# superlinear-ai/raglite

Measured on AMD Instinct MI355X. Metric: queries/sec, MaxSim 32x1M d=1024 exact top-100, higher is better.
Workload: dtype f32 in / f32 scores: candidate chunks found with the fp16 hi halves of corpus and queries (1 x v_mfma_f32_16x16x32_f16 per multiply, f32 accumulate, rigorous error bound), their scores by v_mfma_f32_16x16x4_f32 (exact f32 products); full-precision fallback: 3 x v_mfma_f32_16x16x32_f16 on hi+lo pairs

## Files before the change

### raglite_amd/csrc/maxsim_pp.hip

```cpp
#include <cstdio>
#include <cstdlib>
#include <utility>

#include "common.h"
#include "pp_schedule.h"

namespace rl {

typedef float f32x4 __attribute__((ext_vector_type(4)));
typedef _Float16 h16x8 __attribute__((ext_vector_type(8)));

namespace {
constexpr int PP_RT = 128;
constexpr int PP_NBLK = PP_RT / 16;
constexpr int PP_QPP = 16;
constexpr int PP_DC = 8;
constexpr int PP_LC = 6;
constexpr int PP_CSLOT = PP_NBLK * 1024;
constexpr int PP_STAGE = 1536;
constexpr int PP_LDS = PP_DC * PP_CSLOT + 16 * PP_STAGE * 4;

__device__ __forceinline__ int64_t pp_uniform_i64(int64_t v) {
    const uint32_t lo = __builtin_amdgcn_readfirstlane((uint32_t)(uint64_t)v);
    const uint32_t hi = __builtin_amdgcn_readfirstlane((uint32_t)((uint64_t)v >> 32));
    return (int64_t)(((uint64_t)hi << 32) | lo);
}

enum { PP_HINT_NONE = 0, PP_HINT_NT = 1, PP_HINT_SC1 = 2 };
template <bool NT>
__device__ __forceinline__ void pp_dma(uint32_t lds, const char* src, uint32_t lane16, int hint) {
    const uint32_t l = __builtin_amdgcn_readfirstlane(lds);
    const char* const p = reinterpret_cast<const char*>(pp_uniform_i64(reinterpret_cast<int64_t>(src)));
#ifdef RAGLITE_EXPERIMENTS
    if (!NT && hint == PP_HINT_SC1) {
        asm volatile("s_mov_b32 m0, %0\n\ts_nop 0\n\tglobal_load_lds_dwordx4 %1, %2 sc1" ::"s"(l), "v"(lane16), "s"(p) : "memory", "m0");
        return;
    }
    if (NT || hint == PP_HINT_NT)
#else
    if constexpr (NT)
#endif
        asm volatile("s_mov_b32 m0, %0\n\ts_nop 0\n\tglobal_load_lds_dwordx4 %1, %2 nt" ::"s"(l), "v"(lane16), "s"(p) : "memory", "m0");
    else
        asm volatile("s_mov_b32 m0, %0\n\ts_nop 0\n\tglobal_load_lds_dwordx4 %1, %2" ::"s"(l), "v"(lane16), "s"(p) : "memory", "m0");
}

template <int OFF>
__device__ __forceinline__ void pp_read(f32x4& dst, uint32_t addr) {
    asm volatile("ds_read_b128 %0, %1 offset:%2" : "=v"(dst) : "v"(addr), "n"(OFF) : "memory");
}
__device__ __forceinline__ void pp_pin(f32x4& a, f32x4& b, f32x4& c, f32x4& d) { asm volatile("" : "+v"(a), "+v"(b), "+v"(c), "+v"(d)); }
typedef float f32x16s __attribute__((ext_vector_type(16)));
__device__ __forceinline__ f32x16s pp_sload16(const float* p) {
    f32x16s v;
    const float* const u = reinterpret_cast<const float*>(pp_uniform_i64(reinterpret_cast<int64_t>(p)));
    asm volatile("s_load_dwordx16 %0, %1, 0x0\n\ts_waitcnt lgkmcnt(0)" : "=s"(v) : "s"(u) : "memory");
    return v;
}
__device__ __forceinline__ h16x8 pp_h(const f32x4& v) {
    h16x8 r;
    __builtin_memcpy(&r, &v, 16);
    return r;
}
}

struct PpRows {
    const float* tau;
    const float* q_unscale;
    const float* q_sumsq;
    const float* row_norm;
    const float* blk_minmax;
    int32_t B, QT, metric;
    float* cand_scores; int32_t* cand_ids; uint32_t* cand_cnt; uint32_t* overflow; int32_t cap;
    uint2* log; int32_t log_cap;
    int32_t tile_begin, tile_count;
    float* S; int64_t ld_s; int32_t stride;
    int32_t xcd_passes, dma_hint;
};

template <int DBG, int MODE, bool ROWNORM>
__global__ __launch_bounds__(512, 2) void maxsim_pp_kernel(const char* __restrict__ planes, int64_t n_rows, int32_t nslab,
                                                           const char* __restrict__ qfrag, const float* __restrict__ qmeta, int32_t n_q,
                                                           const int32_t* __restrict__ row_to_chunk, const int64_t* __restrict__ chunk_offsets,
                                                           const uint32_t* __restrict__ ends_bits, float* __restrict__ out, int64_t out_stride,
                                                           float inv_e_scale, const uint32_t* __restrict__ run_if, PpRows rs) {
    constexpr bool ROWS = MODE == 2, SCORES = MODE == 1, GROUPS = ROWS || SCORES;
    __shared__ __attribute__((aligned(16))) char smem[PP_LDS];
    if (run_if && __builtin_amdgcn_readfirstlane((int)*run_if) == 0) return;
    const int lane = threadIdx.x & 63;
    const int wv = wave_id();
    int64_t G = gridDim.x, b = blockIdx.x;
    int qt = (int)blockIdx.y;
    if constexpr (!GROUPS) {
        const int32_t passes = (n_q + PP_QPP - 1) / PP_QPP;
        const PpSlot m = gridDim.y > 1 ? pp_schedule((int32_t)blockIdx.x, (int32_t)blockIdx.y, (int32_t)gridDim.x, (int32_t)gridDim.y, passes)
                                       : pp_schedule_affine((int32_t)blockIdx.x, (int32_t)gridDim.x, passes, rs.xcd_passes);
        G = __builtin_amdgcn_readfirstlane(m.ranges);
        b = __builtin_amdgcn_readfirstlane(m.range);
        qt = __builtin_amdgcn_readfirstlane(m.pass);
    }
    auto boundary = [&](int64_t t) -> int64_t {
        if (t <= 0) return 0;
        if (t >= n_rows) return n_rows;
        const int32_t c = row_to_chunk[t];
        const int64_t c0 = chunk_offsets[c], c1 = chunk_offsets[c + 1];
        return c0 == t ? t : c1;
    };
    int32_t r_lo = 0, r_hi = 0, nt_rows = 0;
    if constexpr (!GROUPS) {
        r_lo = (int32_t)pp_uniform_i64(boundary((n_rows * b) / G));
        r_hi = (int32_t)pp_uniform_i64((b + 1 == G) ? n_rows : boundary((n_rows * (b + 1)) / G));
        if (r_hi <= r_lo) return;
    } else {
        const int64_t Tr = rs.tile_count;
        const int64_t t0 = (Tr * b) / G, t1 = (Tr * (b + 1)) / G;
        nt_rows = (int32_t)(t1 - t0);
        if (nt_rows <= 0) return;
        r_lo = (int32_t)((rs.tile_begin + t0) * PP_RT);
        r_hi = (int32_t)n_rows;
    }
    const int32_t org = r_lo & ~15;
    const int nt = GROUPS ? nt_rows : (r_hi - org + PP_RT - 1) / PP_RT;
    auto tile_blk = [&](int t) __attribute__((always_inline)) -> int32_t {
        if constexpr (SCORES) {
            const int32_t o = (org >> 7) + t;
            return ((o >> 1) * 2 * rs.stride + (o & 1)) * PP_NBLK;
        } else {
            return (org >> 4) + t * PP_NBLK;
        }
    };
    const int q_base = GROUPS ? 0 : PP_QPP * qt;
    const int total = nt * nslab;
    const int32_t last_blk = (int32_t)((n_rows + 15) >> 4) - 1;
    const uint32_t lds_base = (uint32_t)reinterpret_cast<uintptr_t>((__attribute__((address_space(3))) char*)smem);
    const uint32_t lane16 = 16u * lane;

    const bool has0 = q_base + 2 * wv < n_q, has1 = q_base + 2 * wv + 1 < n_q;
    int ql0 = PP_QPP * qt + 2 * wv, ql1 = PP_QPP * qt + 2 * wv + 1;
    ql0 = ql0 < n_q ? ql0 : n_q - 1;
    ql1 = ql1 < n_q ? ql1 : n_q - 1;
    const char* const qp0 = qfrag + pp_uniform_i64((int64_t)ql0 * nslab * 4096);
    const char* const qp1 = qfrag + pp_uniform_i64((int64_t)ql1 * nslab * 4096);
    int qr_s = 0;
    auto issue_qregs = [&](f32x4 (&qn)[4]) __attribute__((always_inline)) {
        if constexpr (!(DBG & 32)) {
            const char* const a0 = reinterpret_cast<const char*>(pp_uniform_i64(reinterpret_cast<int64_t>(qp0 + (int64_t)qr_s * 4096)));
            const char* const a1 = reinterpret_cast<const char*>(pp_uniform_i64(reinterpret_cast<int64_t>(qp1 + (int64_t)qr_s * 4096)));
            asm volatile("global_load_dwordx4 %0, %2, %3\n\tglobal_load_dwordx4 %1, %2, %3 offset:2048"
                         : "=&v"(qn[0]), "=&v"(qn[1]) : "v"(lane16), "s"(a0) : "memory");
            asm volatile("global_load_dwordx4 %0, %2, %3\n\tglobal_load_dwordx4 %1, %2, %3 offset:2048"
                         : "=&v"(qn[2]), "=&v"(qn[3]) : "v"(lane16), "s"(a1) : "memory");
            if (++qr_s == nslab) qr_s = 0;
        }
    };
    int fc_s = 0, fc_r = 0, fc_slot = 0;
    const int dma_hint = GROUPS ? 0 : rs.dma_hint;
    const int32_t blk_org = (org >> 4) + wv;
    const int64_t slab_bytes = (int64_t)nslab * 1024;
    auto issue_c = [&]() __attribute__((always_inline)) {
        if constexpr (!(DBG & 16)) {
            const int t = fc_r < nt ? fc_r : nt - 1;
            int32_t blk = SCORES ? tile_blk(t) + wv : blk_org + t * PP_NBLK;
            blk = blk < last_blk ? blk : last_blk;
            const char* src = planes + pp_uniform_i64((int64_t)blk * slab_bytes + (int64_t)fc_s * 1024);
            pp_dma<GROUPS>(lds_base + (uint32_t)(fc_slot * PP_CSLOT + wv * 1024), src, lane16, dma_hint);
        }
        if (++fc_s == nslab) { fc_s = 0; ++fc_r; }
        fc_slot = fc_slot + 1 == PP_DC ? 0 : fc_slot + 1;
    };

    f32x4 acc[2][2][PP_NBLK];
#pragma unroll
    for (int q = 0; q < 2; ++q)
#pragma unroll
        for (int qb = 0; qb < 2; ++qb)
#pragma unroll
            for (int a = 0; a < PP_NBLK; ++a) acc[q][qb][a] = (f32x4){0.f, 0.f, 0.f, 0.f};

    f32x4 ef[PP_NBLK];
    f32x4 qA[4], qB[4];
    int c_slot = 0;
    const uint32_t rd_c = lds_base + lane16;
    auto read_slab = [&](auto A_) __attribute__((always_inline)) {
        constexpr int a = decltype(A_)::value;
        if constexpr (!(DBG & 8)) pp_read<a * 1024>(ef[a], rd_c + (uint32_t)(c_slot * PP_CSLOT));
    };
    auto mfma_group = [&](f32x4 (&q)[4], auto A_) __attribute__((always_inline)) {
        constexpr int A = decltype(A_)::value;
        if constexpr (!(DBG & 2)) {
            acc[0][0][A] = __builtin_amdgcn_mfma_f32_16x16x32_f16(pp_h(ef[A]), pp_h(q[0]), acc[0][0][A], 0, 0, 0);
            acc[0][1][A] = __builtin_amdgcn_mfma_f32_16x16x32_f16(pp_h(ef[A]), pp_h(q[1]), acc[0][1][A], 0, 0, 0);
            acc[1][0][A] = __builtin_amdgcn_mfma_f32_16x16x32_f16(pp_h(ef[A]), pp_h(q[2]), acc[1][0][A], 0, 0, 0);
            acc[1][1][A] = __builtin_amdgcn_mfma_f32_16x16x32_f16(pp_h(ef[A]), pp_h(q[3]), acc[1][1][A], 0, 0, 0);
        }
    };

    const int fG = lane >> 4, fb = (lane >> 2) & 3, ft = lane & 3;
    const int my_row = (ft >> 1) + 2 * (fb & 1) + 4 * (fb >> 1) + 8 * (fG & 1);
    const uint32_t my_bit = 1u << my_row, my_below = my_bit - 1u;
    float run = -INFINITY;
    uint32_t prev_last_end = 1;
    int32_t ord_run = GROUPS ? 0 : __builtin_amdgcn_readfirstlane(row_to_chunk[org]);
    const int e_q = fG >> 1;
    const bool e_has = !GROUPS && (e_q == 0 ? has0 : has1) && (ft & 1) == 0;
    const float e_unscale = e_has ? qmeta[2 * (q_base + 2 * wv + e_q)] * inv_e_scale : 0.f;
    [[maybe_unused]] float* const o_buf = reinterpret_cast<float*>(smem + PP_DC * PP_CSLOT) + (2 * wv + e_q) * PP_STAGE;
    [[maybe_unused]] const int32_t ord_lo = !GROUPS ? __builtin_amdgcn_readfirstlane(row_to_chunk[r_lo]) : 0;
    [[maybe_unused]] int32_t own_cnt = 0, own_flushed = 0;
    [[maybe_unused]] auto flush_out = [&]() __attribute__((always_inline)) {
        if constexpr (!GROUPS) {
            const int n = own_cnt - own_flushed;
            asm volatile("s_waitcnt lgkmcnt(0)" ::: "memory");
            const float* const b0 = reinterpret_cast<const float*>(smem + PP_DC * PP_CSLOT) + (2 * wv) * PP_STAGE;
            float* const g0 = out + (int64_t)(q_base + 2 * wv) * out_stride + ord_lo + own_flushed;
            if (has0)
                for (int i = lane; i < n; i += 64) g0[i] = b0[i];
            if (has1)
                for (int i = lane; i < n; i += 64) g0[out_stride + i] = b0[PP_STAGE + i];
            own_flushed = own_cnt;
            asm volatile("s_waitcnt vmcnt(0)" ::: "memory");
        }
    };
    const uint64_t odd_pairs = 0xccccccccccccccccull;
    auto swap32 = [](float& x, float& y) __attribute__((always_inline)) {
        const auto r = __builtin_amdgcn_permlane32_swap(__float_as_uint(x), __float_as_uint(y), false, false);
        x = __uint_as_float(r[0]);
        y = __uint_as_float(r[1]);
    };
    auto swap16 = [](float& x, float& y) __attribute__((always_inline)) {
        const auto r = __builtin_amdgcn_permlane16_swap(__float_as_uint(x), __float_as_uint(y), false, false);
        x = __uint_as_float(r[0]);
        y = __uint_as_float(r[1]);
    };
    auto zero_block = [&](auto A_) __attribute__((always_inline)) {
        constexpr int a = decltype(A_)::value;
#pragma unroll
        for (int q = 0; q < 2; ++q)
#pragma unroll
            for (int qb = 0; qb < 2; ++qb) acc[q][qb][a] = (f32x4){0.f, 0.f, 0.f, 0.f};
    };
    [[maybe_unused]] auto block_epilogue_maxsim = [&](auto A_, int T) __attribute__((always_inline)) {
        constexpr int a = decltype(A_)::value;
        const int32_t base = org + T * PP_RT + 16 * a;
        const uint32_t E = (ends_bits[base >> 5] >> (base & 16)) & 0xffffu;
        float z[16];
#pragma unroll
        for (int r = 0; r < 16; ++r) z[r] = acc[r >> 3][(r >> 2) & 1][a][r & 3];
#pragma unroll
        for (int u = 0; u < 4; ++u) { swap32(z[u], z[8 + u]); swap32(z[4 + u], z[12 + u]); }
#pragma unroll
        for (int u = 0; u < 4; ++u) { swap16(z[u], z[4 + u]); swap16(z[8 + u], z[12 + u]); }
        uint64_t saved;
        asm volatile(
            "s_mov_b64 %[sv], exec\n\t"
            "s_bitcmp1_b32 %[ple], 0\n\ts_cselect_b64 exec, 0, -1\n\tv_max_f32 %[z0], %[z0], %[run]\n\t"
            "s_bitcmp1_b32 %[E], 0\n\ts_cselect_b64 exec, 0, -1\n\tv_max_f32 %[z1], %[z1], %[z0]\n\t"
            "s_bitcmp1_b32 %[E], 1\n\ts_cselect_b64 exec, 0, -1\n\tv_max_f32 %[z2], %[z2], %[z1]\n\t"
            "s_bitcmp1_b32 %[E], 2\n\ts_cselect_b64 exec, 0, -1\n\tv_max_f32 %[z3], %[z3], %[z2]\n\t"
            "s_bitcmp1_b32 %[E], 3\n\ts_cselect_b64 exec, 0, -1\n\tv_max_f32 %[z4], %[z4], %[z3]\n\t"
            "s_bitcmp1_b32 %[E], 4\n\ts_cselect_b64 exec, 0, -1\n\tv_max_f32 %[z5], %[z5], %[z4]\n\t"
            "s_bitcmp1_b32 %[E], 5\n\ts_cselect_b64 exec, 0, -1\n\tv_max_f32 %[z6], %[z6], %[z5]\n\t"
            "s_bitcmp1_b32 %[E], 6\n\ts_cselect_b64 exec, 0, -1\n\tv_max_f32 %[z7], %[z7], %[z6]\n\t"
            "s_bitcmp1_b32 %[E], 7\n\ts_cselect_b64 exec, 0, -1\n\tv_max_f32 %[z8], %[z8], %[z7]\n\t"
            "s_bitcmp1_b32 %[E], 8\n\ts_cselect_b64 exec, 0, -1\n\tv_max_f32 %[z9], %[z9], %[z8]\n\t"
            "s_bitcmp1_b32 %[E], 9\n\ts_cselect_b64 exec, 0, -1\n\tv_max_f32 %[z10], %[z10], %[z9]\n\t"
            "s_bitcmp1_b32 %[E], 10\n\ts_cselect_b64 exec, 0, -1\n\tv_max_f32 %[z11], %[z11], %[z10]\n\t"
            "s_bitcmp1_b32 %[E], 11\n\ts_cselect_b64 exec, 0, -1\n\tv_max_f32 %[z12], %[z12], %[z11]\n\t"
            "s_bitcmp1_b32 %[E], 12\n\ts_cselect_b64 exec, 0, -1\n\tv_max_f32 %[z13], %[z13], %[z12]\n\t"
            "s_bitcmp1_b32 %[E], 13\n\ts_cselect_b64 exec, 0, -1\n\tv_max_f32 %[z14], %[z14], %[z13]\n\t"
            "s_bitcmp1_b32 %[E], 14\n\ts_cselect_b64 exec, 0, -1\n\tv_max_f32 %[z15], %[z15], %[z14]\n\t"
            "s_mov_b64 exec, %[sv]"
            : [sv] "=&s"(saved), [z0] "+v"(z[0]), [z1] "+v"(z[1]), [z2] "+v"(z[2]), [z3] "+v"(z[3]), [z4] "+v"(z[4]), [z5] "+v"(z[5]),
              [z6] "+v"(z[6]), [z7] "+v"(z[7]), [z8] "+v"(z[8]), [z9] "+v"(z[9]), [z10] "+v"(z[10]), [z11] "+v"(z[11]), [z12] "+v"(z[12]),
              [z13] "+v"(z[13]), [z14] "+v"(z[14]), [z15] "+v"(z[15])
            : [run] "v"(run), [E] "s"(E), [ple] "s"(prev_last_end)
            : "scc");
        run = z[15];
        prev_last_end = (E >> 15) & 1u;
        float s8[8];
#pragma unroll
        for (int k = 0; k < 8; ++k) {
            swap16(z[k], z[k + 8]);
            s8[k] = z[k] + z[k + 8];
        }
        float t0, t1, w;
        asm volatile(
            "s_nop 1\n\t"
            "v_add_f32_dpp %[s0], %[s0], %[s0] row_ror:8 row_mask:0xf bank_mask:0x3\n\t"
            "v_add_f32_dpp %[s1], %[s1], %[s1] row_ror:8 row_mask:0xf bank_mask:0x3\n\t"
            "v_add_f32_dpp %[s2], %[s2], %[s2] row_ror:8 row_mask:0xf bank_mask:0x3\n\t"
            "v_add_f32_dpp %[s3], %[s3], %[s3] row_ror:8 row_mask:0xf bank_mask:0x3\n\t"
            "v_add_f32_dpp %[s0], %[s4], %[s4] row_ror:8 row_mask:0xf bank_mask:0xc\n\t"
            "v_add_f32_dpp %[s1], %[s5], %[s5] row_ror:8 row_mask:0xf bank_mask:0xc\n\t"
            "v_add_f32_dpp %[s2], %[s6], %[s6] row_ror:8 row_mask:0xf bank_mask:0xc\n\t"
            "v_add_f32_dpp %[s3], %[s7], %[s7] row_ror:8 row_mask:0xf bank_mask:0xc\n\t"
            "v_add_f32_dpp %[s0], %[s0], %[s0] row_shl:4 row_mask:0xf bank_mask:0x5\n\t"
            "v_add_f32_dpp %[s1], %[s1], %[s1] row_shl:4 row_mask:0xf bank_mask:0x5\n\t"
            "v_add_f32_dpp %[s0], %[s2], %[s2] row_shr:4 row_mask:0xf bank_mask:0xa\n\t"
            "v_add_f32_dpp %[s1], %[s3], %[s3] row_shr:4 row_mask:0xf bank_mask:0xa\n\t"
            "s_nop 1\n\t"
            "v_add_f32_dpp %[t0], %[s0], %[s0] quad_perm:[2,3,0,1] row_mask:0xf bank_mask:0xf\n\t"
            "v_add_f32_dpp %[t1], %[s1], %[s1] quad_perm:[2,3,0,1] row_mask:0xf bank_mask:0xf\n\t"
            "v_cndmask_b32_e64 %[w], %[t0], %[t1], %[odd]\n\t"
            "s_nop 1\n\t"
            "v_add_f32_dpp %[w], %[w], %[w] quad_perm:[1,0,3,2] row_mask:0xf bank_mask:0xf"
            : [s0] "+v"(s8[0]), [s1] "+v"(s8[1]), [s2] "+v"(s8[2]), [s3] "+v"(s8[3]), [t0] "=&v"(t0), [t1] "=&v"(t1), [w] "=&v"(w)
            : [s4] "v"(s8[4]), [s5] "v"(s8[5]), [s6] "v"(s8[6]), [s7] "v"(s8[7]), [odd] "s"(odd_pairs));
        int32_t lo = r_lo - base, hi = r_hi - base;
        lo = lo < 0 ? 0 : lo;
        hi = hi < 0 ? 0 : hi;
        asm("" : "+s"(lo), "+s"(hi));
        lo = lo > 16 ? 16 : lo;
        hi = hi > 16 ? 16 : hi;
        uint32_t EM = E & ((1u << hi) - 1u) & ~((1u << lo) - 1u);
        asm("" : "+s"(EM));
        if (EM != 0u) {
            if ((EM & my_bit) && e_has) o_buf[ord_run - ord_lo - own_flushed + __builtin_popcount(E & my_below)] = w * e_unscale;
            own_cnt += __builtin_popcount(EM);
        }
        ord_run += __builtin_popcount(E);
        zero_block(A_);
    };

    [[maybe_unused]] float T4x = INFINITY;
    [[maybe_unused]] uint32_t ncand = 0;
    constexpr uint32_t LOG_CAP = PP_STAGE;
    [[maybe_unused]] uint2* const l_log = reinterpret_cast<uint2*>(smem + PP_DC * PP_CSLOT) + wv * LOG_CAP;
    [[maybe_unused]] uint32_t ncand_out = 0;
    [[maybe_unused]] uint2* const my_log = ROWS ? rs.log + (((size_t)blockIdx.y * gridDim.x + blockIdx.x) * 8 + wv) * (size_t)rs.log_cap : nullptr;
    [[maybe_unused]] const bool cosine = GROUPS && rs.metric == SCAN_COSINE;
    [[maybe_unused]] float Ux = 0.f, Rx = 0.f;
    if constexpr (SCORES) {
        const int c = lane >> 4;
        const int32_t q = (16 * qt + 2 * wv + (c >> 1)) * 32 + 16 * (c & 1) + (lane & 15);
        const int32_t qc = q < rs.B ? q : rs.B - 1;
        Ux = q < rs.B ? rs.q_unscale[qc] * inv_e_scale : 0.f;
        Rx = cosine ? 1.0f / sqrtf(rs.q_sumsq[qc]) : 1.0f;
    }
    if constexpr (ROWS) {
        const int c = lane >> 4;
        const int32_t q = (16 * qt + 2 * wv + (c >> 1)) * 32 + 16 * (c & 1) + (lane & 15);
        const int32_t qc = q < rs.B ? q : rs.B - 1;
        const float us = rs.q_unscale[qc] * inv_e_scale;
        const float tq = rs.tau[qc];
        const bool bad = q < rs.B && !(tq > -INFINITY);
        const float slack = 1e-5f * fmaxf(1.0f, fabsf(tq));
        const float t_dot = cosine ? (tq - slack) * sqrtf(rs.q_sumsq[qc]) : (tq - 1.0f) - slack;
        T4x = q < rs.B ? (t_dot - fabsf(t_dot) * 1e-6f) / us : INFINITY;
        if (__builtin_amdgcn_ballot_w64(bad) != 0 && lane == 0) *rs.overflow = 1u;
    }
    [[maybe_unused]] auto rows_thresholds = [&](float (&tq4)[4]) __attribute__((always_inline)) {
        uint32_t b;
        asm volatile("v_mbcnt_lo_u32_b32 %0, -1, 0\n\tv_mbcnt_hi_u32_b32 %0, -1, %0" : "=v"(b));
        b = (b & 15u) << 2;
#pragma unroll
        for (int c = 0; c < 4; ++c)
            tq4[c] = __int_as_float(__builtin_amdgcn_ds_bpermute((int)(((uint32_t)c << 6) | b), __float_as_int(T4x)));
    };
    [[maybe_unused]] auto block_epilogue_rows = [&](auto A_, int T, const float (&tq4)[4], float nmin, float nmax) __attribute__((always_inline)) {
        constexpr int a = decltype(A_)::value;
        const int32_t base = org + T * PP_RT + 16 * a;
        if (base < (int32_t)n_rows) {
            uint32_t lane_code = ((uint32_t)(lane & 15) << 7) | (uint32_t)(4 * (lane >> 4));
            asm volatile("" : "+v"(lane_code));
            float t4[4];
#pragma unroll
            for (int c = 0; c < 4; ++c) t4[c] = tq4[c];
            if (cosine) {
                nmin *= 0.999999f;
                nmax *= 1.000001f;
#pragma unroll
                for (int c = 0; c < 4; ++c) t4[c] = fminf(t4[c] * nmin, t4[c] * nmax);
            }
            const uint32_t code_a = ((uint32_t)T << 13) | (uint32_t)(16 * a);
            if constexpr (ROWNORM) {
                float top4[4];
                bool any_hit = false;
#pragma unroll
                for (int c = 0; c < 4; ++c) {
                    const f32x4 v4 = acc[c >> 1][c & 1][a];
                    top4[c] = fmaxf(fmaxf(v4[0], v4[1]), fmaxf(v4[2], v4[3]));
                    any_hit |= __builtin_amdgcn_ballot_w64(top4[c] >= t4[c]) != 0ull;
                }
                float nv0 = 1.f, nv1 = 1.f, nv2 = 1.f, nv3 = 1.f;
                const bool row_norms = cosine && base + 16 <= (int32_t)n_rows;
                if (any_hit && row_norms) {
                    const f32x16s nr = pp_sload16(rs.row_norm + base);
                    const int gq = lane >> 4;
                    nv0 = gq == 0 ? nr[0] : gq == 1 ? nr[4] : gq == 2 ? nr[8] : nr[12];
                    nv1 = gq == 0 ? nr[1] : gq == 1 ? nr[5] : gq == 2 ? nr[9] : nr[13];
                    nv2 = gq == 0 ? nr[2] : gq == 1 ? nr[6] : gq == 2 ? nr[10] : nr[14];
                    nv3 = gq == 0 ? nr[3] : gq == 1 ? nr[7] : gq == 2 ? nr[11] : nr[15];
                }
#pragma unroll
                for (int c = 0; c < 4; ++c) {
                    const f32x4 v4 = acc[c >> 1][c & 1][a];
                    if (__builtin_amdgcn_ballot_w64(top4[c] >= t4[c]) != 0ull) {
                        float r0 = v4[0], r1 = v4[1], r2 = v4[2], r3 = v4[3];
                        const float tc = tq4[c];
                        float n0 = nv0, n1 = nv1, n2 = nv2, n3 = nv3;
                        if (cosine && !row_norms) n0 = n1 = n2 = n3 = tc >= 0.f ? nmin : nmax;
                        uint32_t code = (code_a + ((uint32_t)c << 11)) | lane_code;
#pragma nounroll
// ... 61 lines not shown
            f32x4 o4;
#pragma unroll
            for (int u = 0; u < 4; ++u) {
                const float d = v4[u] * us4[c];
                float v = cosine ? 1.0f - (1.0f - d * rn[u] * rq4[c]) : 1.0f + d;
                o4[u] = u < left ? v : -INFINITY;
            }
            const int32_t q = (16 * qt + 2 * wv + (c >> 1)) * 32 + 16 * (c & 1) + (int32_t)n_op;
            if (q < rs.B) *reinterpret_cast<f32x4*>(rs.S + (int64_t)q * rs.ld_s + col + 4 * gq) = o4;
        }
        zero_block(A_);
    };
    [[maybe_unused]] auto dump_log = [&]() __attribute__((always_inline)) {
        if constexpr (ROWS) {
            uint32_t n = ncand - ncand_out;
            if (n > LOG_CAP) {
                if (lane == 0) *rs.overflow = 1u;
                n = LOG_CAP;
            }
            asm volatile("s_waitcnt lgkmcnt(0)" ::: "memory");
            for (uint32_t i = lane; i < n; i += 64)
                if (ncand_out + i < (uint32_t)rs.log_cap) my_log[ncand_out + i] = l_log[i];
            ncand_out = ncand;
            asm volatile("s_waitcnt vmcnt(0)" ::: "memory");
        }
    };
    [[maybe_unused]] auto flush_rows = [&]() __attribute__((always_inline)) {
        if constexpr (ROWS) {
            if (ncand > (uint32_t)rs.log_cap) {
                if (lane == 0) *rs.overflow = 1u;
                ncand = (uint32_t)rs.log_cap;
            }
            const int mode = rs.metric;
            for (uint32_t i = lane; i < ncand; i += 64) {
                const uint2 rec = my_log[i];
                const uint32_t m = rec.y;
                const int T = (int)(m >> 13), c = (int)((m >> 11) & 3u), n = (int)((m >> 7) & 15u), r = (int)(m & 127u);
                const int32_t q = (16 * qt + 2 * wv + (c >> 1)) * 32 + 16 * (c & 1) + n, row = org + T * PP_RT + r;
                if (q >= rs.B || row >= (int32_t)n_rows) continue;
                const float d = __uint_as_float(rec.x) * (rs.q_unscale[q] * inv_e_scale);
                float v = d;
                if (mode == SCAN_COSINE) v = 1.0f - (1.0f - d / (rs.row_norm[row] * sqrtf(rs.q_sumsq[q])));
                else if (mode == SCAN_DOT) v = 1.0f + d;
                if (!(v >= rs.tau[q])) continue;
                const uint32_t slot = atomicAdd(rs.cand_cnt + q, 1u);
                if (slot < (uint32_t)rs.cap) {
                    rs.cand_scores[(int64_t)q * rs.cap + slot] = v;
                    rs.cand_ids[(int64_t)q * rs.cap + slot] = row;
                } else {
                    *rs.overflow = 1u;
                }
            }
        }
    };

    int c_s = 0, c_r = 0;
#define PP_I(N) std::integral_constant<int, N>{}
    auto tile_end = [&]() __attribute__((always_inline)) {
        if constexpr (DBG & 128) return;
        if (c_s == nslab - 1) {
            if constexpr (SCORES) {
                float us4[4], rq4[4];
                uint32_t bl;
                asm volatile("v_mbcnt_lo_u32_b32 %0, -1, 0\n\tv_mbcnt_hi_u32_b32 %0, -1, %0" : "=v"(bl));
                bl = (bl & 15u) << 2;
#pragma unroll
                for (int c = 0; c < 4; ++c) {
                    us4[c] = __int_as_float(__builtin_amdgcn_ds_bpermute((int)(((uint32_t)c << 6) | bl), __float_as_int(Ux)));
                    rq4[c] = __int_as_float(__builtin_amdgcn_ds_bpermute((int)(((uint32_t)c << 6) | bl), __float_as_int(Rx)));
                }
                [&]<int... A>(std::integer_sequence<int, A...>) {
                    (block_epilogue_scores(std::integral_constant<int, A>{}, c_r, us4, rq4, bl >> 2), ...);
                }(std::make_integer_sequence<int, PP_NBLK>{});
            } else if constexpr (ROWS) {
                float tq4[4];
                rows_thresholds(tq4);
                f32x16s mm = {};
                if (cosine) mm = pp_sload16(rs.blk_minmax + 2 * ((org + c_r * PP_RT) >> 4));
                [&]<int... A>(std::integer_sequence<int, A...>) {
                    (block_epilogue_rows(std::integral_constant<int, A>{}, c_r, tq4, mm[2 * A], mm[2 * A + 1]), ...);
                }(std::make_integer_sequence<int, PP_NBLK>{});
                if (ncand - ncand_out > LOG_CAP / 2) dump_log();
            } else {
                [&]<int... A>(std::integer_sequence<int, A...>) { (block_epilogue_maxsim(std::integral_constant<int, A>{}, c_r), ...); }
                (std::make_integer_sequence<int, PP_NBLK>{});
                if (own_cnt - own_flushed > PP_STAGE - PP_RT) flush_out();
            }
        }
    };
    auto slab = [&](f32x4 (&q)[4], f32x4 (&qn)[4], auto LAG_) __attribute__((always_inline)) {
        constexpr bool LAG = decltype(LAG_)::value;
        auto G = [&](auto A_) __attribute__((always_inline)) { mfma_group(q, A_); };
        auto R = [&](auto A_) __attribute__((always_inline)) { read_slab(A_); };
        issue_qregs(qn);
        issue_c();
        __builtin_amdgcn_sched_barrier(0);
        if constexpr (!LAG) {
            G(PP_I(0)); R(PP_I(0)); __builtin_amdgcn_sched_barrier(0);
            G(PP_I(1)); R(PP_I(1)); __builtin_amdgcn_sched_barrier(0);
            G(PP_I(2)); R(PP_I(2)); __builtin_amdgcn_sched_barrier(0);
            G(PP_I(3)); R(PP_I(3)); __builtin_amdgcn_sched_barrier(0);
            asm volatile("s_waitcnt lgkmcnt(4)" ::: "memory");
        } else {
            G(PP_I(0)); __builtin_amdgcn_sched_barrier(0);
            G(PP_I(1)); R(PP_I(0)); __builtin_amdgcn_sched_barrier(0);
            G(PP_I(2)); R(PP_I(1)); __builtin_amdgcn_sched_barrier(0);
            G(PP_I(3)); R(PP_I(2)); __builtin_amdgcn_sched_barrier(0);
            asm volatile("s_waitcnt lgkmcnt(3)" ::: "memory");
        }
        pp_pin(ef[4], ef[5], ef[6], ef[7]);
        asm volatile("s_barrier" ::: "memory");
        __builtin_amdgcn_sched_barrier(0);
        if constexpr (!LAG) {
            G(PP_I(4)); R(PP_I(4)); __builtin_amdgcn_sched_barrier(0);
            G(PP_I(5)); R(PP_I(5)); __builtin_amdgcn_sched_barrier(0);
            G(PP_I(6)); R(PP_I(6)); __builtin_amdgcn_sched_barrier(0);
            G(PP_I(7)); R(PP_I(7)); __builtin_amdgcn_sched_barrier(0);
        } else {
            G(PP_I(4)); R(PP_I(3)); __builtin_amdgcn_sched_barrier(0);
            G(PP_I(5)); R(PP_I(4)); __builtin_amdgcn_sched_barrier(0);
            G(PP_I(6)); R(PP_I(5)); __builtin_amdgcn_sched_barrier(0);
            G(PP_I(7)); R(PP_I(6)); __builtin_amdgcn_sched_barrier(0);
            R(PP_I(7)); __builtin_amdgcn_sched_barrier(0);
        }
        c_slot = c_slot + 1 == PP_DC ? 0 : c_slot + 1;
        tile_end();
        if (++c_s == nslab) { c_s = 0; ++c_r; }
    };
    auto landed = [&](f32x4 (&qn)[4]) __attribute__((always_inline)) {
        asm volatile("s_waitcnt lgkmcnt(4)" ::: "memory");
        asm volatile("s_waitcnt vmcnt(1)" ::: "memory");
        pp_pin(ef[0], ef[1], ef[2], ef[3]);
        pp_pin(qn[0], qn[1], qn[2], qn[3]);
    };

    for (int i = 0; i < PP_LC; ++i) issue_c();
    issue_qregs(qA);
    asm volatile("s_waitcnt vmcnt(0)\n\ts_barrier" ::: "memory");
    [&]<int... A>(std::integer_sequence<int, A...>) { (read_slab(std::integral_constant<int, A>{}), ...); }
    (std::make_integer_sequence<int, PP_NBLK>{});
    c_slot = 1;
    landed(qA);
    auto main_loop = [&](auto LAG_) __attribute__((always_inline)) {
        for (int g = 0; g < total; g += 2) {
            slab(qA, qB, LAG_);
            landed(qB);
            if (g + 1 < total) {
                slab(qB, qA, LAG_);
                landed(qA);
            }
        }
    };
#undef PP_I
    if (wv < 4) main_loop(std::false_type{});
    else main_loop(std::true_type{});
    asm volatile("s_waitcnt vmcnt(0)" ::: "memory");
    dump_log();
    flush_rows();
    flush_out();
    if constexpr (DBG & 128) {
        if (n_q > 1000000) {
            f32x4 t = (f32x4){0.f, 0.f, 0.f, 0.f};
#pragma unroll
            for (int q = 0; q < 2; ++q)
#pragma unroll
                for (int qb = 0; qb < 2; ++qb)
#pragma unroll
                    for (int a = 0; a < PP_NBLK; ++a) t += acc[q][qb][a];
            out[lane] = (t[0] + t[1]) + (t[2] + t[3]);
        }
    }
}

int launch_maxsim_pp(const void* image, int64_t n_rows, int32_t dim, const void* qbuf, int32_t n_queries, int32_t first, int32_t n_q,
                     int32_t nq, const int32_t* row_to_chunk, const int64_t* chunk_offsets, const uint32_t* ends_bits, float* out,
                     int64_t out_stride, int n_cu, hipStream_t s, float split_scale, const uint32_t* run_if, int schedule, int xcd_passes) {
    if (nq < 1 || nq > 32 || n_q < 1 || n_q > PP_QPP * 4096 || n_rows < 1 || first < 0 || first + n_q > n_queries) return RL_ERR_UNSUPPORTED;
    if (dim % 32 || dim < 256 || !(split_scale > 0.f) || !image || !ends_bits) return RL_ERR_UNSUPPORTED;
    const int32_t nslab = dim / 32;
    const char* qfrag = static_cast<const char*>(qbuf) + (size_t)first * nslab * 4096;
    const float* qmeta = reinterpret_cast<const float*>(static_cast<const char*>(qbuf) + (size_t)n_queries * dim * 128) + 2 * (size_t)first;
    const int64_t tiles = (n_rows + PP_RT - 1) / PP_RT;
    const int64_t gx = std::max<int64_t>(1, std::min<int64_t>(n_cu > 0 ? n_cu : 256, tiles)), passes = (n_q + PP_QPP - 1) / PP_QPP;
    const dim3 grid = schedule == 1 ? dim3((unsigned)(gx * passes)) : dim3((unsigned)gx, (unsigned)passes), blk(512);
    PpRows rs{};
    rs.xcd_passes = schedule == 1 ? xcd_passes : 8;
#define RL_PP_LAUNCH(DBG_)                                                                                                                 \
    hipLaunchKernelGGL((maxsim_pp_kernel<DBG_, 0, false>), grid, blk, 0, s, static_cast<const char*>(image), n_rows, nslab, qfrag, qmeta, n_q, row_to_chunk, \
                       chunk_offsets, ends_bits, out, out_stride, 1.0f / split_scale, run_if, rs)
#ifdef RAGLITE_EXPERIMENTS
    const int force_hint = std::getenv("RAGLITE_PP_HINT") ? std::atoi(std::getenv("RAGLITE_PP_HINT")) : -1;
    if (force_hint >= PP_HINT_NONE && force_hint <= PP_HINT_SC1) rs.dma_hint = force_hint;
    static const int dbg = std::getenv("RAGLITE_PP_DBG") ? std::atoi(std::getenv("RAGLITE_PP_DBG")) : 0;
    if (dbg == 2) RL_PP_LAUNCH(2);
    else if (dbg == 128) RL_PP_LAUNCH(128);
    else if (dbg == 136) RL_PP_LAUNCH(136);
    else if (dbg == 144) RL_PP_LAUNCH(144);
    else if (dbg == 160) RL_PP_LAUNCH(160);
    else if (dbg == 184) RL_PP_LAUNCH(184);
    else RL_PP_LAUNCH(0);
#else
    RL_PP_LAUNCH(0);
#endif
#undef RL_PP_LAUNCH
    RL_HIP(hipGetLastError());
    return RL_OK;
}

__global__ __launch_bounds__(256) void block_norm_minmax_kernel(const float* __restrict__ row_norm, int64_t n_rows, int64_t n_blocks,
                                                                 float* __restrict__ out) {
    const int64_t blk = (int64_t)blockIdx.x * 256 + threadIdx.x;
    if (blk >= n_blocks) return;
    float mn = INFINITY, mx = 0.f;
    for (int i = 0; i < 16; ++i) {
        const int64_t r = blk * 16 + i;
        if (r < n_rows) { const float v = row_norm[r]; mn = fminf(mn, v); mx = fmaxf(mx, v); }
    }
    out[2 * blk] = mn;
    out[2 * blk + 1] = mx;
}

int launch_pp_rows_sample(const void* image, int64_t n_rows, int32_t dim, int32_t nb, float* scratch, const float* row_norm, int mode, float* S,
                          int64_t ld_s, int32_t stride, int n_cu, hipStream_t s, float split_scale) {
    if (nb < 1 || n_rows < 1 || dim % 32 || dim < 256 || !(split_scale > 0.f) || !image || !S || stride < 1) return RL_ERR_UNSUPPORTED;
    if (mode != SCAN_COSINE && mode != SCAN_DOT) return RL_ERR_UNSUPPORTED;
    if (mode == SCAN_COSINE && !row_norm) return RL_ERR_INVALID;
    if ((ld_s & 255) || (reinterpret_cast<uintptr_t>(S) & 15)) return RL_ERR_UNSUPPORTED;
    const int32_t nslab = dim / 32, groups = (nb + 31) / 32;
    float* frag = scratch;
    float* unscale = frag + (size_t)groups * 32 * dim;
    float* anylo = unscale + nb;
    float* qss = anylo + groups;
    const int64_t grid_cu = n_cu > 0 ? n_cu : 256;
    const int64_t T256 = (n_rows + 255) / 256, Tv = (T256 + stride - 1) / stride;
    if (Tv * 256 != ld_s) return RL_ERR_INVALID;
    PpRows rs{};
    rs.tile_begin = 0;
    rs.tile_count = (int32_t)(2 * Tv);
    rs.q_unscale = unscale; rs.q_sumsq = qss; rs.row_norm = row_norm; rs.B = nb; rs.QT = (groups + PP_QPP - 1) / PP_QPP; rs.metric = mode;
    rs.S = S; rs.ld_s = ld_s; rs.stride = stride;
    if (rs.QT > grid_cu) return RL_ERR_UNSUPPORTED;
    const int64_t gx = std::max<int64_t>(1, std::min<int64_t>(grid_cu / rs.QT, 2 * Tv));
    hipLaunchKernelGGL((maxsim_pp_kernel<0, 1, false>), dim3((unsigned)gx, (unsigned)rs.QT), dim3(512), 0, s, static_cast<const char*>(image), n_rows,
                       nslab, reinterpret_cast<const char*>(frag), nullptr, groups, nullptr, nullptr, nullptr, nullptr, (int64_t)0,
                       1.0f / split_scale, nullptr, rs);
    RL_HIP(hipGetLastError());
    return RL_OK;
}

size_t pp_rows_scratch_bytes(int64_t n_rows, int32_t nb, int n_cu, int32_t expected_per_query, int32_t* log_cap_out) {
    const int64_t grid = n_cu > 0 ? n_cu : 256;
    int64_t cap = ((int64_t)expected_per_query * nb * 4) / (grid * 8) + 1;
    cap = std::max<int64_t>(4096, (cap + 1023) & ~int64_t(1023));
    cap = std::min<int64_t>(cap, int64_t(1) << 19);
    if (log_cap_out) *log_cap_out = (int32_t)cap;
    const size_t blocks = (size_t)((n_rows + 15) / 16);
    return (size_t)grid * 8 * (size_t)cap * sizeof(uint2) + blocks * 2 * sizeof(float) + 256;
}

int launch_pp_rows_pass(const void* image, int64_t n_rows, int32_t dim, int32_t nb, float* scratch, const float* row_norm, int mode,
                        const CandArgs* cand, void* work, int32_t log_cap, int n_cu, hipStream_t s, float split_scale, int64_t tile_begin,
                        int64_t tile_count, bool norms_ready, bool row_norm_test) {
    if (nb < 1 || n_rows < 1 || dim % 32 || dim < 256 || !(split_scale > 0.f) || !image || !cand || !work) return RL_ERR_UNSUPPORTED;
    if (mode != SCAN_COSINE && mode != SCAN_DOT) return RL_ERR_UNSUPPORTED;
    if (mode == SCAN_COSINE && !row_norm) return RL_ERR_INVALID;
    if (cand->tau_stride != 1) return RL_ERR_UNSUPPORTED;
    const int32_t nslab = dim / 32, groups = (nb + 31) / 32;
    float* frag = scratch;
    float* unscale = frag + (size_t)groups * 32 * dim;
    float* anylo = unscale + nb;
    float* qss = anylo + groups;
    const int64_t grid_cu = n_cu > 0 ? n_cu : 256;
    const int64_t Tr_all = (n_rows + PP_RT - 1) / PP_RT;
    if (tile_count < 0) tile_count = Tr_all - tile_begin;
    if (tile_begin < 0 || tile_count < 1 || tile_begin + tile_count > Tr_all) return RL_ERR_INVALID;
    const int64_t Tr = tile_count;
    PpRows rs{};
    rs.tile_begin = (int32_t)tile_begin;
    rs.tile_count = (int32_t)tile_count;
    rs.tau = cand->tau; rs.q_unscale = unscale; rs.q_sumsq = qss; rs.row_norm = row_norm; rs.B = nb; rs.QT = (groups + PP_QPP - 1) / PP_QPP;
    rs.metric = mode; rs.cand_scores = cand->scores; rs.cand_ids = cand->ids; rs.cand_cnt = cand->cnt; rs.overflow = cand->overflow; rs.cap = cand->cap;
    rs.log = static_cast<uint2*>(work);
    rs.log_cap = log_cap;
    if (rs.QT > grid_cu || Tr_all + 2 >= (int64_t(1) << 19)) return RL_ERR_UNSUPPORTED;
    float* blk_mm = reinterpret_cast<float*>(static_cast<char*>(work) + (size_t)grid_cu * 8 * (size_t)log_cap * sizeof(uint2));
    rs.blk_minmax = blk_mm;
    if (mode == SCAN_COSINE && !norms_ready) {
// ... 70 lines not shown
```

Baseline: 18140.

## Stage per-chunk maxima in LDS and reduce in batches instead of per-block DPP reductions

The per-block 16-row DPP cross-lane sum is replaced. Each chunk end now writes its per-lane running maxima to an LDS staging area, and a batched reduce_staged pass sums up to 32 staged chunks at once with ds_read_b32. The ends bits for a whole tile come from one scalar s_load_dwordx8 instead of per-block global loads. The exec-mask segmented max chain is simplified with s_bfe_i64 on a precomputed mask, and tile_end is skipped in the even slab when nslab is even, with a MODE 3 variant used for odd nslab. This aims to cut VALU and DPP work in the epilogue, at the cost of extra LDS traffic and a smaller output buffer that flushes more often.

```diff
diff --git a/raglite_amd/csrc/maxsim_pp.hip b/raglite_amd/csrc/maxsim_pp.hip
--- a/raglite_amd/csrc/maxsim_pp.hip
+++ b/raglite_amd/csrc/maxsim_pp.hip
@@ -19,6 +19,10 @@
 constexpr int PP_CSLOT = PP_NBLK * 1024;
 constexpr int PP_STAGE = 1536;
 constexpr int PP_LDS = PP_DC * PP_CSLOT + 16 * PP_STAGE * 4;
+constexpr int PP_SSLOTS = 32;
+constexpr int PP_SPITCH = 65;
+constexpr int PP_OCAP = 496;
+static_assert(2 * PP_OCAP + (PP_SSLOTS - 1) * PP_SPITCH + 64 <= 2 * PP_STAGE, "a wave's results and staging area share its 12 KiB");
 
 __device__ __forceinline__ int64_t pp_uniform_i64(int64_t v) {
     const uint32_t lo = __builtin_amdgcn_readfirstlane((uint32_t)(uint64_t)v);
@@ -56,6 +60,18 @@
     const float* const u = reinterpret_cast<const float*>(pp_uniform_i64(reinterpret_cast<int64_t>(p)));
     asm volatile("s_load_dwordx16 %0, %1, 0x0\n\ts_waitcnt lgkmcnt(0)" : "=s"(v) : "s"(u) : "memory");
     return v;
+}
+typedef uint32_t u32x8s __attribute__((ext_vector_type(8)));
+__device__ __forceinline__ u32x8s pp_sload8(const uint32_t* p) {
+    u32x8s v;
+    const uint32_t* const u = reinterpret_cast<const uint32_t*>(pp_uniform_i64(reinterpret_cast<int64_t>(p)));
+    asm volatile("s_load_dwordx8 %0, %1, 0x0\n\ts_waitcnt lgkmcnt(0)" : "=s"(v) : "s"(u) : "memory");
+    return v;
+}
+__device__ __forceinline__ void pp_write1(uint32_t addr, float v) { asm volatile("ds_write_b32 %0, %1" ::"v"(addr), "v"(v) : "memory"); }
+template <int OFF>
+__device__ __forceinline__ void pp_read1(float& dst, uint32_t addr) {
+    asm volatile("ds_read_b32 %0, %1 offset:%2" : "=v"(dst) : "v"(addr), "n"(OFF) : "memory");
 }
 __device__ __forceinline__ h16x8 pp_h(const f32x4& v) {
     h16x8 r;
@@ -85,6 +101,7 @@
                                                            const uint32_t* __restrict__ ends_bits, float* __restrict__ out, int64_t out_stride,
                                                            float inv_e_scale, const uint32_t* __restrict__ run_if, PpRows rs) {
     constexpr bool ROWS = MODE == 2, SCORES = MODE == 1, GROUPS = ROWS || SCORES;
+    constexpr bool TILE_END_IN_BOTH = MODE != 0;
     __shared__ __attribute__((aligned(16))) char smem[PP_LDS];
     if (run_if && __builtin_amdgcn_readfirstlane((int)*run_if) == 0) return;
     const int lane = threadIdx.x & 63;
@@ -195,33 +212,69 @@
         }
     };
 
-    const int fG = lane >> 4, fb = (lane >> 2) & 3, ft = lane & 3;
-    const int my_row = (ft >> 1) + 2 * (fb & 1) + 4 * (fb >> 1) + 8 * (fG & 1);
-    const uint32_t my_bit = 1u << my_row, my_below = my_bit - 1u;
     float run = -INFINITY;
     uint32_t prev_last_end = 1;
-    int32_t ord_run = GROUPS ? 0 : __builtin_amdgcn_readfirstlane(row_to_chunk[org]);
-    const int e_q = fG >> 1;
-    const bool e_has = !GROUPS && (e_q == 0 ? has0 : has1) && (ft & 1) == 0;
-    const float e_unscale = e_has ? qmeta[2 * (q_base + 2 * wv + e_q)] * inv_e_scale : 0.f;
-    [[maybe_unused]] float* const o_buf = reinterpret_cast<float*>(smem + PP_DC * PP_CSLOT) + (2 * wv + e_q) * PP_STAGE;
+    [[maybe_unused]] uint32_t e_us0 = 0u, e_us1 = 0u;
+    if constexpr (!GROUPS) {
+        e_us0 = __builtin_amdgcn_readfirstlane(has0 ? __float_as_uint(qmeta[2 * (q_base + 2 * wv)] * inv_e_scale) : 0u);
+        e_us1 = __builtin_amdgcn_readfirstlane(has1 ? __float_as_uint(qmeta[2 * (q_base + 2 * wv + 1)] * inv_e_scale) : 0u);
+    }
+    [[maybe_unused]] const uint32_t w_lds = (uint32_t)__builtin_amdgcn_readfirstlane((int)(lds_base + (uint32_t)(PP_DC * PP_CSLOT + wv * (2 * PP_STAGE * 4))));
+    [[maybe_unused]] const uint32_t st_lds = w_lds + 2 * PP_OCAP * 4;
+    [[maybe_unused]] uint32_t lane4 = lane16;
+    if constexpr (!GROUPS) asm volatile("v_lshrrev_b32 %0, 2, %0" : "+v"(lane4));
     [[maybe_unused]] const int32_t ord_lo = !GROUPS ? __builtin_amdgcn_readfirstlane(row_to_chunk[r_lo]) : 0;
-    [[maybe_unused]] int32_t own_cnt = 0, own_flushed = 0;
+    [[maybe_unused]] int32_t own_cnt = 0, n_st = 0, own_flushed = 0;
     [[maybe_unused]] auto flush_out = [&]() __attribute__((always_inline)) {
         if constexpr (!GROUPS) {
-            const int n = own_cnt - own_flushed;
+            const int n = own_cnt - n_st - own_flushed;
             asm volatile("s_waitcnt lgkmcnt(0)" ::: "memory");
             const float* const b0 = reinterpret_cast<const float*>(smem + PP_DC * PP_CSLOT) + (2 * wv) * PP_STAGE;
             float* const g0 = out + (int64_t)(q_base + 2 * wv) * out_stride + ord_lo + own_flushed;
+            int ln;
+            asm volatile("v_mbcnt_lo_u32_b32 %0, -1, 0\n\tv_mbcnt_hi_u32_b32 %0, -1, %0" : "=v"(ln));
             if (has0)
-                for (int i = lane; i < n; i += 64) g0[i] = b0[i];
+#pragma nounroll
+                for (int i = ln; i < n; i += 64) g0[i] = b0[i];
             if (has1)
-                for (int i = lane; i < n; i += 64) g0[out_stride + i] = b0[PP_STAGE + i];
-            own_flushed = own_cnt;
+#pragma nounroll
+                for (int i = ln; i < n; i += 64) g0[out_stride + i] = b0[PP_OCAP + i];
+            own_flushed += n;
             asm volatile("s_waitcnt vmcnt(0)" ::: "memory");
         }
     };
-    const uint64_t odd_pairs = 0xccccccccccccccccull;
+    [[maybe_unused]] auto reduce_staged = [&]() __attribute__((always_inline)) {
+        if constexpr (!GROUPS) {
+            uint32_t ln;
+            asm volatile("v_mbcnt_lo_u32_b32 %0, -1, 0\n\tv_mbcnt_hi_u32_b32 %0, -1, %0" : "=v"(ln));
+            const uint32_t slot = ln & (uint32_t)(PP_SSLOTS - 1), q = ln >> 5;
+            uint32_t ra = st_lds + slot * (PP_SPITCH * 4) + q * 128;
+            float w = 0.f;
+#pragma nounroll
+            for (int h = 0; h < 2; ++h) {
+                float s0[8], s1[8];
+                [&]<int... J>(std::integer_sequence<int, J...>) { ((pp_read1<8 * J>(s0[J], ra), pp_read1<8 * J + 64>(s1[J], ra)), ...); }
+                (std::make_integer_sequence<int, 8>{});
+                asm volatile("s_waitcnt lgkmcnt(0)" ::: "memory");
+#pragma unroll
+                for (int j = 0; j < 8; ++j) asm volatile("" : "+v"(s0[j]), "+v"(s1[j]));
+                float p[8];
+#pragma unroll
+                for (int j = 0; j < 8; ++j) p[j] = s0[j] + s1[j];
+                const float a0 = p[0] + p[4], a1 = p[1] + p[5], a2 = p[2] + p[6], a3 = p[3] + p[7];
+                const float c = (a0 + a2) + (a1 + a3);
+                w = h == 0 ? c : w + c;
+                ra += 4;
+                asm volatile("" : "+v"(ra), "+v"(w));
+            }
+            uint32_t u0 = e_us0, u1 = e_us1;
+            asm volatile("" : "+s"(u0), "+s"(u1));
+            const bool has = q == 0 ? has0 : has1;
+            float* const o = reinterpret_cast<float*>(smem + PP_DC * PP_CSLOT) + (2 * wv) * PP_STAGE + q * PP_OCAP;
+            if (has && (int32_t)slot < n_st) o[own_cnt - n_st - own_flushed + (int32_t)slot] = w * __uint_as_float(q == 0 ? u0 : u1);
+            n_st = 0;
+        }
+    };
     auto swap32 = [](float& x, float& y) __attribute__((always_inline)) {
         const auto r = __builtin_amdgcn_permlane32_swap(__float_as_uint(x), __float_as_uint(y), false, false);
         x = __uint_as_float(r[0]);
@@ -239,10 +292,11 @@
 #pragma unroll
             for (int qb = 0; qb < 2; ++qb) acc[q][qb][a] = (f32x4){0.f, 0.f, 0.f, 0.f};
     };
-    [[maybe_unused]] auto block_epilogue_maxsim = [&](auto A_, int T) __attribute__((always_inline)) {
+    [[maybe_unused]] auto block_epilogue_maxsim = [&](auto A_, int T, uint32_t Ew) __attribute__((always_inline)) {
         constexpr int a = decltype(A_)::value;
         const int32_t base = org + T * PP_RT + 16 * a;
-        const uint32_t E = (ends_bits[base >> 5] >> (base & 16)) & 0xffffu;
+        uint32_t E = (Ew >> (16 * (a & 1))) & 0xffffu;
+        asm("" : "+s"(E));
         float z[16];
 #pragma unroll
         for (int r = 0; r < 16; ++r) z[r] = acc[r >> 3][(r >> 2) & 1][a][r & 3];
@@ -250,62 +304,36 @@
         for (int u = 0; u < 4; ++u) { swap32(z[u], z[8 + u]); swap32(z[4 + u], z[12 + u]); }
 #pragma unroll
         for (int u = 0; u < 4; ++u) { swap16(z[u], z[4 + u]); swap16(z[8 + u], z[12 + u]); }
+        uint32_t nm = ~((E << 1) | prev_last_end);
+        asm("" : "+s"(nm));
+        const uint64_t nM = nm;
         uint64_t saved;
         asm volatile(
             "s_mov_b64 %[sv], exec\n\t"
-            "s_bitcmp1_b32 %[ple], 0\n\ts_cselect_b64 exec, 0, -1\n\tv_max_f32 %[z0], %[z0], %[run]\n\t"
-            "s_bitcmp1_b32 %[E], 0\n\ts_cselect_b64 exec, 0, -1\n\tv_max_f32 %[z1], %[z1], %[z0]\n\t"
-            "s_bitcmp1_b32 %[E], 1\n\ts_cselect_b64 exec, 0, -1\n\tv_max_f32 %[z2], %[z2], %[z1]\n\t"
-            "s_bitcmp1_b32 %[E], 2\n\ts_cselect_b64 exec, 0, -1\n\tv_max_f32 %[z3], %[z3], %[z2]\n\t"
-            "s_bitcmp1_b32 %[E], 3\n\ts_cselect_b64 exec, 0, -1\n\tv_max_f32 %[z4], %[z4], %[z3]\n\t"
-            "s_bitcmp1_b32 %[E], 4\n\ts_cselect_b64 exec, 0, -1\n\tv_max_f32 %[z5], %[z5], %[z4]\n\t"
-            "s_bitcmp1_b32 %[E], 5\n\ts_cselect_b64 exec, 0, -1\n\tv_max_f32 %[z6], %[z6], %[z5]\n\t"
-            "s_bitcmp1_b32 %[E], 6\n\ts_cselect_b64 exec, 0, -1\n\tv_max_f32 %[z7], %[z7], %[z6]\n\t"
-            "s_bitcmp1_b32 %[E], 7\n\ts_cselect_b64 exec, 0, -1\n\tv_max_f32 %[z8], %[z8], %[z7]\n\t"
-            "s_bitcmp1_b32 %[E], 8\n\ts_cselect_b64 exec, 0, -1\n\tv_max_f32 %[z9], %[z9], %[z8]\n\t"
-            "s_bitcmp1_b32 %[E], 9\n\ts_cselect_b64 exec, 0, -1\n\tv_max_f32 %[z10], %[z10], %[z9]\n\t"
-            "s_bitcmp1_b32 %[E], 10\n\ts_cselect_b64 exec, 0, -1\n\tv_max_f32 %[z11], %[z11], %[z10]\n\t"
-            "s_bitcmp1_b32 %[E], 11\n\ts_cselect_b64 exec, 0, -1\n\tv_max_f32 %[z12], %[z12], %[z11]\n\t"
-            "s_bitcmp1_b32 %[E], 12\n\ts_cselect_b64 exec, 0, -1\n\tv_max_f32 %[z13], %[z13], %[z12]\n\t"
-            "s_bitcmp1_b32 %[E], 13\n\ts_cselect_b64 exec, 0, -1\n\tv_max_f32 %[z14], %[z14], %[z13]\n\t"
-            "s_bitcmp1_b32 %[E], 14\n\ts_cselect_b64 exec, 0, -1\n\tv_max_f32 %[z15], %[z15], %[z14]\n\t"
+            "s_bfe_i64 exec, %[nM], 0x10000\n\tv_max_f32 %[z0], %[z0], %[run]\n\t"
+            "s_bfe_i64 exec, %[nM], 0x10001\n\tv_max_f32 %[z1], %[z1], %[z0]\n\t"
+            "s_bfe_i64 exec, %[nM], 0x10002\n\tv_max_f32 %[z2], %[z2], %[z1]\n\t"
+            "s_bfe_i64 exec, %[nM], 0x10003\n\tv_max_f32 %[z3], %[z3], %[z2]\n\t"
+            "s_bfe_i64 exec, %[nM], 0x10004\n\tv_max_f32 %[z4], %[z4], %[z3]\n\t"
+            "s_bfe_i64 exec, %[nM], 0x10005\n\tv_max_f32 %[z5], %[z5], %[z4]\n\t"
+            "s_bfe_i64 exec, %[nM], 0x10006\n\tv_max_f32 %[z6], %[z6], %[z5]\n\t"
+            "s_bfe_i64 exec, %[nM], 0x10007\n\tv_max_f32 %[z7], %[z7], %[z6]\n\t"
+            "s_bfe_i64 exec, %[nM], 0x10008\n\tv_max_f32 %[z8], %[z8], %[z7]\n\t"
+            "s_bfe_i64 exec, %[nM], 0x10009\n\tv_max_f32 %[z9], %[z9], %[z8]\n\t"
+            "s_bfe_i64 exec, %[nM], 0x1000a\n\tv_max_f32 %[z10], %[z10], %[z9]\n\t"
+            "s_bfe_i64 exec, %[nM], 0x1000b\n\tv_max_f32 %[z11], %[z11], %[z10]\n\t"
+            "s_bfe_i64 exec, %[nM], 0x1000c\n\tv_max_f32 %[z12], %[z12], %[z11]\n\t"
+            "s_bfe_i64 exec, %[nM], 0x1000d\n\tv_max_f32 %[z13], %[z13], %[z12]\n\t"
+            "s_bfe_i64 exec, %[nM], 0x1000e\n\tv_max_f32 %[z14], %[z14], %[z13]\n\t"
+            "s_bfe_i64 exec, %[nM], 0x1000f\n\tv_max_f32 %[z15], %[z15], %[z14]\n\t"
             "s_mov_b64 exec, %[sv]"
             : [sv] "=&s"(saved), [z0] "+v"(z[0]), [z1] "+v"(z[1]), [z2] "+v"(z[2]), [z3] "+v"(z[3]), [z4] "+v"(z[4]), [z5] "+v"(z[5]),
               [z6] "+v"(z[6]), [z7] "+v"(z[7]), [z8] "+v"(z[8]), [z9] "+v"(z[9]), [z10] "+v"(z[10]), [z11] "+v"(z[11]), [z12] "+v"(z[12]),
               [z13] "+v"(z[13]), [z14] "+v"(z[14]), [z15] "+v"(z[15])
-            : [run] "v"(run), [E] "s"(E), [ple] "s"(prev_last_end)
+            : [run] "v"(run), [nM] "s"(nM)
             : "scc");
         run = z[15];
         prev_last_end = (E >> 15) & 1u;
-        float s8[8];
-#pragma unroll
-        for (int k = 0; k < 8; ++k) {
-            swap16(z[k], z[k + 8]);
-            s8[k] = z[k] + z[k + 8];
-        }
-        float t0, t1, w;
-        asm volatile(
-            "s_nop 1\n\t"
-            "v_add_f32_dpp %[s0], %[s0], %[s0] row_ror:8 row_mask:0xf bank_mask:0x3\n\t"
-            "v_add_f32_dpp %[s1], %[s1], %[s1] row_ror:8 row_mask:0xf bank_mask:0x3\n\t"
-            "v_add_f32_dpp %[s2], %[s2], %[s2] row_ror:8 row_mask:0xf bank_mask:0x3\n\t"
-            "v_add_f32_dpp %[s3], %[s3], %[s3] row_ror:8 row_mask:0xf bank_mask:0x3\n\t"
-            "v_add_f32_dpp %[s0], %[s4], %[s4] row_ror:8 row_mask:0xf bank_mask:0xc\n\t"
-            "v_add_f32_dpp %[s1], %[s5], %[s5] row_ror:8 row_mask:0xf bank_mask:0xc\n\t"
-            "v_add_f32_dpp %[s2], %[s6], %[s6] row_ror:8 row_mask:0xf bank_mask:0xc\n\t"
-            "v_add_f32_dpp %[s3], %[s7], %[s7] row_ror:8 row_mask:0xf bank_mask:0xc\n\t"
-            "v_add_f32_dpp %[s0], %[s0], %[s0] row_shl:4 row_mask:0xf bank_mask:0x5\n\t"
-            "v_add_f32_dpp %[s1], %[s1], %[s1] row_shl:4 row_mask:0xf bank_mask:0x5\n\t"
-            "v_add_f32_dpp %[s0], %[s2], %[s2] row_shr:4 row_mask:0xf bank_mask:0xa\n\t"
-            "v_add_f32_dpp %[s1], %[s3], %[s3] row_shr:4 row_mask:0xf bank_mask:0xa\n\t"
-            "s_nop 1\n\t"
-            "v_add_f32_dpp %[t0], %[s0], %[s0] quad_perm:[2,3,0,1] row_mask:0xf bank_mask:0xf\n\t"
-            "v_add_f32_dpp %[t1], %[s1], %[s1] quad_perm:[2,3,0,1] row_mask:0xf bank_mask:0xf\n\t"
-            "v_cndmask_b32_e64 %[w], %[t0], %[t1], %[odd]\n\t"
-            "s_nop 1\n\t"
-            "v_add_f32_dpp %[w], %[w], %[w] quad_perm:[1,0,3,2] row_mask:0xf bank_mask:0xf"
-            : [s0] "+v"(s8[0]), [s1] "+v"(s8[1]), [s2] "+v"(s8[2]), [s3] "+v"(s8[3]), [t0] "=&v"(t0), [t1] "=&v"(t1), [w] "=&v"(w)
-            : [s4] "v"(s8[4]), [s5] "v"(s8[5]), [s6] "v"(s8[6]), [s7] "v"(s8[7]), [odd] "s"(odd_pairs));
         int32_t lo = r_lo - base, hi = r_hi - base;
         lo = lo < 0 ? 0 : lo;
         hi = hi < 0 ? 0 : hi;
@@ -315,10 +343,22 @@
         uint32_t EM = E & ((1u << hi) - 1u) & ~((1u << lo) - 1u);
         asm("" : "+s"(EM));
         if (EM != 0u) {
-            if ((EM & my_bit) && e_has) o_buf[ord_run - ord_lo - own_flushed + __builtin_popcount(E & my_below)] = w * e_unscale;
-            own_cnt += __builtin_popcount(EM);
-        }
-        ord_run += __builtin_popcount(E);
+            uint32_t so = st_lds + (uint32_t)n_st * (PP_SPITCH * 4);
+#pragma unroll
+            for (int r4 = 0; r4 < 16; r4 += 4)
+                if (EM & (0xfu << r4)) {
+#pragma unroll
+                    for (int r = r4; r < r4 + 4; ++r)
+                        if (EM & (1u << r)) {
+                            pp_write1(so + lane4, z[r]);
+                            so += PP_SPITCH * 4;
+                        }
+                }
+            const int32_t ne = __builtin_popcount(EM);
+            own_cnt += ne;
+            n_st += ne;
+            if (n_st > PP_SSLOTS - 16) reduce_staged();
+        }
         zero_block(A_);
     };
 
@@ -546,14 +586,20 @@
                 }(std::make_integer_sequence<int, PP_NBLK>{});
                 if (ncand - ncand_out > LOG_CAP / 2) dump_log();
             } else {
-                [&]<int... A>(std::integer_sequence<int, A...>) { (block_epilogue_maxsim(std::integral_constant<int, A>{}, c_r), ...); }
+                const int32_t tb = org + c_r * PP_RT;
+                const u32x8s eb = pp_sload8(ends_bits + (tb >> 5));
+                const uint32_t sh = (uint32_t)tb & 16u;
+                const uint32_t Ew[4] = {(uint32_t)((((uint64_t)eb[1] << 32) | eb[0]) >> sh), (uint32_t)((((uint64_t)eb[2] << 32) | eb[1]) >> sh),
+                                        (uint32_t)((((uint64_t)eb[3] << 32) | eb[2]) >> sh), (uint32_t)((((uint64_t)eb[4] << 32) | eb[3]) >> sh)};
+                if (own_cnt - own_flushed + __builtin_popcount(Ew[0]) + __builtin_popcount(Ew[1]) + __builtin_popcount(Ew[2]) + __builtin_popcount(Ew[3]) > PP_OCAP)
+                    flush_out();
+                [&]<int... A>(std::integer_sequence<int, A...>) { (block_epilogue_maxsim(std::integral_constant<int, A>{}, c_r, Ew[A >> 1]), ...); }
                 (std::make_integer_sequence<int, PP_NBLK>{});
-                if (own_cnt - own_flushed > PP_STAGE - PP_RT) flush_out();
             }
         }
     };
-    auto slab = [&](f32x4 (&q)[4], f32x4 (&qn)[4], auto LAG_) __attribute__((always_inline)) {
-        constexpr bool LAG = decltype(LAG_)::value;
+    auto slab = [&](f32x4 (&q)[4], f32x4 (&qn)[4], auto LAG_, auto TE_) __attribute__((always_inline)) {
+        constexpr bool LAG = decltype(LAG_)::value, TE = decltype(TE_)::value;
         auto G = [&](auto A_) __attribute__((always_inline)) { mfma_group(q, A_); };
         auto R = [&](auto A_) __attribute__((always_inline)) { read_slab(A_); };
         issue_qregs(qn);
@@ -588,7 +634,7 @@
             R(PP_I(7)); __builtin_amdgcn_sched_barrier(0);
         }
         c_slot = c_slot + 1 == PP_DC ? 0 : c_slot + 1;
-        tile_end();
+        if constexpr (TE) tile_end();
         if (++c_s == nslab) { c_s = 0; ++c_r; }
     };
     auto landed = [&](f32x4 (&qn)[4]) __attribute__((always_inline)) {
@@ -607,10 +653,10 @@
     landed(qA);
     auto main_loop = [&](auto LAG_) __attribute__((always_inline)) {
         for (int g = 0; g < total; g += 2) {
-            slab(qA, qB, LAG_);
+            slab(qA, qB, LAG_, std::bool_constant<TILE_END_IN_BOTH>{});
             landed(qB);
             if (g + 1 < total) {
-                slab(qB, qA, LAG_);
+                slab(qB, qA, LAG_, std::true_type{});
                 landed(qA);
             }
         }
@@ -621,7 +667,10 @@
     asm volatile("s_waitcnt vmcnt(0)" ::: "memory");
     dump_log();
     flush_rows();
-    flush_out();
+    if constexpr (!GROUPS) {
+        if (n_st > 0) reduce_staged();
+        flush_out();
+    }
     if constexpr (DBG & 128) {
         if (n_q > 1000000) {
             f32x4 t = (f32x4){0.f, 0.f, 0.f, 0.f};
@@ -649,9 +698,14 @@
     const dim3 grid = schedule == 1 ? dim3((unsigned)(gx * passes)) : dim3((unsigned)gx, (unsigned)passes), blk(512);
     PpRows rs{};
     rs.xcd_passes = schedule == 1 ? xcd_passes : 8;
+#define RL_PP_LAUNCH_(DBG_, MODE_)                                                                                                         \
+    hipLaunchKernelGGL((maxsim_pp_kernel<DBG_, MODE_, false>), grid, blk, 0, s, static_cast<const char*>(image), n_rows, nslab, qfrag, qmeta, n_q, row_to_chunk, \
+                       chunk_offsets, ends_bits, out, out_stride, 1.0f / split_scale, run_if, rs)
 #define RL_PP_LAUNCH(DBG_)                                                                                                                 \
-    hipLaunchKernelGGL((maxsim_pp_kernel<DBG_, 0, false>), grid, blk, 0, s, static_cast<const char*>(image), n_rows, nslab, qfrag, qmeta, n_q, row_to_chunk, \
-                       chunk_offsets, ends_bits, out, out_stride, 1.0f / split_scale, run_if, rs)
+    do {                                                                                                                                   \
+        if (nslab & 1) RL_PP_LAUNCH_(DBG_, 3);                                                                                             \
+        else RL_PP_LAUNCH_(DBG_, 0);                                                                                                       \
+    } while (0)
 #ifdef RAGLITE_EXPERIMENTS
     const int force_hint = std::getenv("RAGLITE_PP_HINT") ? std::atoi(std::getenv("RAGLITE_PP_HINT")) : -1;
     if (force_hint >= PP_HINT_NONE && force_hint <= PP_HINT_SC1) rs.dma_hint = force_hint;
@@ -667,6 +721,7 @@
     RL_PP_LAUNCH(0);
 #endif
 #undef RL_PP_LAUNCH
+#undef RL_PP_LAUNCH_
     RL_HIP(hipGetLastError());
     return RL_OK;
 }
```

Result: no change. 18260 (median of 6 runs) (+0.6%).
